# asheptunov/graph-neural-net

Measured on AMD Instinct MI355X. Metric: training samples/sec, 784-300-100-10 MLP batch 128, higher is better.
Workload: dtype f32; 1 GPU; 784-300-100-10 SoftmaxCrossEntropyNeuralNet gradientStep, fp32, batch 128 per GPU (BASELINE configs[1]); global_batch=128, parallelism=dp1, inner_activation=leaky_relu

## Files before the change

graph-neural-net_amd/csrc/abi.hip:

```cpp
#include "handle.h"
#include "confusion_kernel.h"

#include <algorithm>

#include <chrono>
#include "java_random.h"

#include <cmath>
#include <cstdio>
#include <cstdlib>
#include <cstring>

using namespace gnn;
using namespace gnn::host;

namespace {
thread_local std::string g_last_error;
void read_env(gnn_mlp *h) {
    auto is = [](const char *name, const char *val) { const char *e = getenv(name); return e && !strcmp(e, val); };
    h->env_path = is("GNN_MLP_PATH", "generic") ? 1 : is("GNN_MLP_PATH", "nomid4") ? 2 : 0;
    const char *hy = getenv("GNN_MLP_HYBRID");
    h->env_hybrid = hy ? (atoi(hy) & 3) : -1;
    h->env_tail_off = is("GNN_MLP_TAIL", "0");
    h->env_graph = is("GNN_MLP_GRAPH", "1");
    h->env_jit_off = is("GNN_MLP_JIT", "0");
    h->env_static_off = is("GNN_MLP_STATIC", "0");
    h->env_chain_off = is("GNN_MLP_CHAIN", "0");
    h->env_wavek_off = is("GNN_MLP_WAVEK", "0");
    h->env_bf16_dma_off = is("GNN_MLP_BF16_DMA", "0");
    h->env_f32_dma_off = is("GNN_MLP_F32_DMA", "0");
    h->env_bf16_group_off = is("GNN_MLP_BF16_GROUP", "0");
    h->env_rb_off = is("GNN_MLP_ROWBLOCK", "0");
    h->env_defer_off = is("GNN_MLP_DEFER", "0");
    const char *fg = getenv("GNN_MLP_FIRST_GEMM_ROWS");
    if (fg) h->first_gemm_rows = atoi(fg);
    const char *fw = getenv("GNN_MLP_FIRST_WAVEK_ROWS");
    if (fw) h->first_wavek_rows = atoi(fw);
    const char *er = getenv("GNN_MLP_EVAL_ROWS");
    if (er) h->eval_rows_cap = atoi(er);
}
}

namespace gnn {
namespace host {

thread_local ArenaCarve *t_arena = nullptr;

int dev_bytes(void **p, size_t bytes) {
    ArenaCarve *a = t_arena;
    if (a && !a->record) {
        const size_t at = (a->used + 255) & ~(size_t)255;
        if (at + bytes > a->cap) { *p = nullptr; return fail(GNN_ERR_STATE, "group arena exhausted: the members' allocations differ"); }
        *p = a->base + at;
        a->used = at + bytes;
        return GNN_OK;
    }
    HIP_TRY(hipMalloc(p, bytes));
    if (a) a->used = ((a->used + 255) & ~(size_t)255) + bytes;
    return GNN_OK;
}
void dev_release(gnn_mlp *h, void *p) {
    if (!p) return;
    if (h->arena_lo && (size_t)(static_cast<char *>(p) - h->arena_lo) < h->arena_bytes) return;
    (void)hipFree(p);
}
// ... 743 lines not shown
```

graph-neural-net_amd/csrc/group_kernels.h:

```cpp
#pragma once
#include "rowblock_kernel.h"
#include "tile_step_kernel.h"

namespace gnn {

constexpr int GROUP_MAX = 16;

struct GroupArgs {
    const char *arena_lo;
    unsigned long long S;
    const char *idx_lo;
    unsigned long long idx_S;
    int nbx;
    float step_over_b[GROUP_MAX];
    float momentum[GROUP_MAX];
};
struct GroupRows {
    int rows[GROUP_MAX];
    int next_rows[GROUP_MAX];
};

template <class T> __device__ __forceinline__ T *group_rel(T *q, const GroupArgs &g, unsigned long long shift) {
    const unsigned long long d = (unsigned long long)reinterpret_cast<const char *>(q) - (unsigned long long)g.arena_lo;
    return d < g.S ? reinterpret_cast<T *>((unsigned long long)q + shift) : q;
}
__device__ __forceinline__ const int32_t *group_rel_idx(const int32_t *q, const GroupArgs &g, unsigned long long shift) {
    const unsigned long long a = (unsigned long long)reinterpret_cast<const char *>(q);
    const unsigned long long in_idx = 0ull - (unsigned long long)(a - (unsigned long long)g.idx_lo < g.idx_S);
    const unsigned long long in_arena = 0ull - (unsigned long long)(a - (unsigned long long)g.arena_lo < g.S);
    return reinterpret_cast<const int32_t *>(a + ((in_idx & ((unsigned long long)blockIdx.y * g.idx_S)) | (~in_idx & in_arena & shift)));
}
struct GroupIdx { const int32_t *row0, *row, *next; };
template <class T> __device__ __forceinline__ T *group_rel(T *q, const GroupArgs &g, unsigned long long shift, const GroupIdx &) { return group_rel(q, g, shift); }
__device__ __forceinline__ const int32_t *group_rel(const int32_t *q, const GroupArgs &, unsigned long long, const GroupIdx &ix) { return q == ix.row0 ? ix.row : ix.next; }

#define TS_BID blockIdx.x
#define TS_REL(q) group_rel((q), ga, ga_shift, ga_idx)
#define TS_REL_LAYER(L) (L.A = TS_REL(L.A), L.D = TS_REL(L.D), L.W = TS_REL(L.W), L.V = TS_REL(L.V), L.G = TS_REL(L.G))
#define TS_STEP_OVER_B ga.step_over_b[blockIdx.y]
#define TS_MOMENTUM ga.momentum[blockIdx.y]
#define TS_K p.K
#define TS_K_TRUE p.k_true
#define TS_NEXT_ROWS p.next_rows
#define TS_NEXT_K p.next_K
template <int GSRC, int GDST, bool FWD>
__global__ __launch_bounds__(TS_THREADS) void tile_step_group_kernel(TileStepParams p, GroupArgs ga) {
    static_assert(GSRC <= 2, "grouped tile kernels: single-GPU forms only");
    const unsigned long long ga_shift = (unsigned long long)blockIdx.y * ga.S;
    const GroupIdx ga_idx{p.row_idx, group_rel_idx(p.row_idx, ga, ga_shift), group_rel_idx(p.next_idx, ga, ga_shift)};
#include "tile_step_body.inc"
}
template <int GSRC, int GDST, bool FWD>
__global__ __launch_bounds__(TS_THREADS) void tile_step_bf16_group_kernel(TileStepParams p, GroupArgs ga) {
    static_assert(GSRC <= 2, "grouped tile kernels: single-GPU forms only");
    const unsigned long long ga_shift = (unsigned long long)blockIdx.y * ga.S;
    const GroupIdx ga_idx{p.row_idx, group_rel_idx(p.row_idx, ga, ga_shift), group_rel_idx(p.next_idx, ga, ga_shift)};
#include "tile_step_bf16_body.inc"
}
#undef TS_K
#undef TS_K_TRUE
#undef TS_NEXT_ROWS
#undef TS_NEXT_K
#define TS_K ga_K
#define TS_K_TRUE ga_k_true
#define TS_NEXT_ROWS ga_next_rows
#define TS_NEXT_K ga_next_K
#define GNN_GROUP_ROW_COUNTS                                                                      \
    const int ga_k_true = gr.rows[blockIdx.y], ga_K = pad_up(ga_k_true);                          \
    const int ga_next_rows = gr.next_rows[blockIdx.y], ga_next_K = pad_up(ga_next_rows);          \
    (void)ga_k_true; (void)ga_K; (void)ga_next_rows; (void)ga_next_K;
template <int GSRC, int GDST, bool FWD>
__global__ __launch_bounds__(TS_THREADS) void tile_step_group_sized_kernel(TileStepParams p, GroupArgs ga, GroupRows gr) {
    static_assert(GSRC <= 2, "grouped tile kernels: single-GPU forms only");
    const unsigned long long ga_shift = (unsigned long long)blockIdx.y * ga.S;
    const GroupIdx ga_idx{p.row_idx, group_rel_idx(p.row_idx, ga, ga_shift), group_rel_idx(p.next_idx, ga, ga_shift)};
    GNN_GROUP_ROW_COUNTS
#include "tile_step_body.inc"
}
template <int GSRC, int GDST, bool FWD>
__global__ __launch_bounds__(TS_THREADS) void tile_step_bf16_group_sized_kernel(TileStepParams p, GroupArgs ga, GroupRows gr) {
    static_assert(GSRC <= 2, "grouped tile kernels: single-GPU forms only");
    const unsigned long long ga_shift = (unsigned long long)blockIdx.y * ga.S;
    const GroupIdx ga_idx{p.row_idx, group_rel_idx(p.row_idx, ga, ga_shift), group_rel_idx(p.next_idx, ga, ga_shift)};
    GNN_GROUP_ROW_COUNTS
#include "tile_step_bf16_body.inc"
}
#undef TS_BID
#undef TS_REL
#undef TS_REL_LAYER
#undef TS_STEP_OVER_B
#undef TS_MOMENTUM
#undef TS_K
#undef TS_K_TRUE
#undef TS_NEXT_ROWS
#undef TS_NEXT_K
#undef GNN_GROUP_ROW_COUNTS

#define GNN_RB_GROUP_MEMBER(ROWS)                                                                                                  \
    const unsigned long long sh = (unsigned long long)blockIdx.y * g.S;                                                            \
    p.slabs = group_rel(slabs, g, sh); p.row_idx = group_rel_idx(row_idx, g, sh); p.copy_idx = group_rel_idx(copy_idx, g, sh);     \
    _Pragma("unroll")                                                                                                              \
    for (int l = 0; l < MAX_LAYERS; l++) {                                                                                         \
        p.W[l] = group_rel(p.W[l], g, sh); p.act[l] = group_rel(p.act[l], g, sh); p.delta[l] = group_rel(p.delta[l], g, sh);       \
        p.Wb[l] = group_rel(p.Wb[l], g, sh); p.actb[l] = group_rel(p.actb[l], g, sh); p.deltab[l] = group_rel(p.deltab[l], g, sh); \
    }                                                                                                                              \
    p.prob = group_rel(p.prob, g, sh); p.loss = group_rel(p.loss, g, sh); p.label = group_rel(p.label, g, sh);                     \
    p.xcopy = group_rel(p.xcopy, g, sh); p.xcopyb = group_rel(p.xcopyb, g, sh);                                                    \
    p.X = group_rel(p.X, g, sh); p.Xb = group_rel(p.Xb, g, sh);                                                                    \
    if constexpr (BF) {                                                                                                            \
        p.Wb[1] = group_rel(reinterpret_cast<const __bf16 *>(W1), g, sh);                                                          \
        if constexpr (SH::kL > 0) p.Wb[SH::kL - 2] = group_rel(reinterpret_cast<const __bf16 *>(Wlast), g, sh);                    \
    } else {                                                                                                                       \
        p.W[1] = group_rel(W1, g, sh);                                                                                             \
        if constexpr (SH::kL > 0) p.W[SH::kL - 2] = group_rel(Wlast, g, sh);                                                       \
    }                                                                                                                              \
    p.Y = group_rel(Y, g, sh); p.B = (ROWS); p.slab_rows = slab_rows; p.ldy = ldy;                                                 \
    if constexpr (SH::is_static) {                                                                                                 \
        constexpr RbPlan m = SH::make();                                                                                           \
        static_assert(m.ok, "this shape does not fit the row-block kernel");                                                       \
// ... 22 lines not shown
```

graph-neural-net_amd/csrc/handle.h:

```cpp
#pragma once
#include "../../include/gnn_mlp.h"
#include "fused_kernels.h"
#include "gemm_bf16.h"
#include "gemm_wavek.h"
#include "middle4_kernel.h"
#include "rowblock_kernel.h"
#include "tile_step_kernel.h"
#include "group_kernels.h"
#include "group_eval_kernel.h"
#include "kernels.h"
#include "eval_kernels.h"
#include "lookahead.h"
#include "group_sizes.h"
#include "timer_slots.h"

#include <hip/hip_ext.h>
#include <hip/hip_runtime.h>

#include <cstdint>
#include <cstring>
#include <exception>
#include <new>
#include <string>
#include <vector>
// ... 41 lines not shown

    float *DX = nullptr, *DY = nullptr;
    __bf16 *Wb = nullptr;
    std::vector<__bf16 *> actb, deltab;
    __bf16 *DXb = nullptr;
    int64_t dataset_n = 0;

    hipStream_t stream = nullptr, own_stream = nullptr;

    bool fused = false;
    gnn::GradParams grad{};
    int grad_tiles = 0;
    gnn::GradParams grad64{};
    int grad_tiles64 = 0;
    bool mid_generic = false;
    bool mid4 = false;
    gnn::Mid4Params mid4p{};
    size_t mid4_lds_bytes = 0;
    const void *mid4_fn[3] = {nullptr, nullptr, nullptr};
    hipFunction_t mid4_jit[3] = {nullptr, nullptr, nullptr};

    bool rb = false;
    gnn::RbParams rbp{};
    size_t rb_lds_bytes = 0;
    const void *rb_fn = nullptr;
    hipFunction_t rb_jit = nullptr;
    int rb_static = 0;

    bool chain = false;
    gnn::TileStepParams tsp{};
    int ts_tiles = 0, ts_tiles0 = 0;
    uint32_t *ts_map = nullptr, *ts_map0 = nullptr;
    bool ts_map_args = false; uint32_t ts_map_words[2][gnn::TS_MAP_ARGS / 2];
    float *slabs = nullptr;
    int n_slabs = 0;
    std::string plan_note;
    gnn::host::Lookahead la;
    float *xstage[2] = {nullptr, nullptr}; __bf16 *xstage_b[2] = {nullptr, nullptr};
    int specialization = 0;
    bool jit_tried = false;
    int steps_seen = 0;

    hipGraphExec_t tr_exec = nullptr;
    hipGraph_t tr_graph = nullptr;
    int64_t tr_first_batch = -1; int tr_B = 0; int64_t tr_nb = 0; double tr_step = 0, tr_mom = 0;
    const float *tr_dx = nullptr;

    struct PendingUpdate { bool on = false; int B = 0; float step_over_b = 0.f, momentum = 0.f; } pend;
    float *act0_alt = nullptr;
    bool env_defer_off = false;

    static constexpr int kEvalRows = 16384;
    int eval_rows_cap = kEvalRows;
    struct EvalWorkspace {
        int rows = 0;
        std::vector<float *> act;
        float *logits = nullptr, *prob = nullptr, *lossv = nullptr;
        int32_t *labels = nullptr;
    } evalws;

    void *rccl_comm = nullptr; int rccl_ranks = 0, rccl_rank = 0;

    gnn_mlp_group *group = nullptr;
    const gnn::host::GroupLaunch *grp = nullptr;
    char *arena_lo = nullptr; size_t arena_bytes = 0;
    bool shared_dataset = false;
    bool shared_stream = false;

    hipError_t launch_error = hipSuccess;
    const int32_t *cur_idx = nullptr;

    bool timing = false;
    TimerClass timers[5];

    int env_path = 0;
    int env_hybrid = -1;
    bool env_tail_off = false;
    bool env_f32_dma_off = false;
    bool env_bf16_group_off = false;
    bool env_bf16_dma_off = false;
    bool env_wavek_off = false;
    bool env_graph = false;
    bool env_jit_off = false;
    bool env_static_off = false;
    bool env_chain_off = false;
    int first_wavek_rows = 256;
    int first_gemm_rows = 2048;
    bool env_rb_off = false;
};

struct gnn_mlp_group {
    int K = 0, device = 0;
    hipStream_t stream = nullptr;
    char *arena = nullptr;
    size_t S = 0;
    std::vector<gnn_mlp *> m;
    bool grouped = false;
    const void *rb_fn = nullptr;
    const void *rb_fn_sized = nullptr;
    struct EvalPlan { bool ok = false; int mt = 0; gnn::GroupEvalLds lds{}; const void *fn = nullptr, *fn_loss = nullptr; } eval_plan;
    float *eval_ws = nullptr;
    int eval_ws_rows = 0;
    int64_t each_grouped = 0, each_mixed = 0;
    gnn::host::GroupSizes sizes;
};

namespace gnn {
namespace host {

void plan_group_eval(gnn_mlp_group *g);
void free_group_eval(gnn_mlp_group *g);
int enqueue_group_validation(gnn_mlp_group *g, int n, float *loss_rows, int64_t stride);
int enqueue_group_curve_sum(gnn_mlp_group *g, const float *rows, int n_rows, int64_t stride, int n, double *d_out);

int fail(int code, const std::string &msg);
const char *last_error_message();
int check_launches(gnn_mlp *h);
int check_handle(gnn_mlp *h, bool apply_pending = true);
int check_batch(const gnn_mlp *h, int B);
int check_range(const gnn_mlp *h, int64_t first, int B);
// ... 206 lines not shown
```

graph-neural-net_amd/csrc/launch_small.hip:

```cpp
#include "static_shapes.h"
#include "jit.h"

using namespace gnn;
using namespace gnn::host;

namespace gnn {
namespace host {

template <class SH> bool shape_matches(const gnn_mlp *h) {
    constexpr int n = (int)(sizeof(SH::kDims) / sizeof(int));
    if (h->L != n) return false;
    for (int i = 0; i < n; i++) if (h->dims[i] != SH::kDims[i]) return false;
    return true;
}

int static_shape_of(const gnn_mlp *h) {
    if (h->env_static_off) return -1;
    if (shape_matches<ShapeMnistA>(h)) return 0;
    if (shape_matches<ShapeMnistB>(h)) return 1;
    return -1;
}

const void *mid4_function(const gnn_mlp *h, int variant) {
    const bool softmax = h->out_kind == GNN_OUT_SOFTMAX_CE;
// ... 94 lines not shown
void fused_forward(gnn_mlp *h, const float *a0, const float *y, int B, bool backward, bool want_prob,
                   bool want_loss, bool want_label, bool from_slabs, int copy_rows) {
    if (!from_slabs) launch_fwd_first(h, a0, B);
    if (from_slabs && h->rb) {
        RbParams r = h->rbp;
        bind_call(h, r, y, B, want_prob, want_loss, want_label);
        if (copy_rows == RB_COPY_CURRENT && h->cur_idx) {
            r.ldx = h->ld[0]; r.copy_idx = h->cur_idx;
            if (h->dtype == GNN_DTYPE_BF16) { r.Xb = a0_bf16(h, a0); r.xcopyb = h->xstage_b[h->la.xstage_cur]; }
            else { r.X = a0; r.xcopy = h->xstage[h->la.xstage_cur]; }
        } else if (copy_rows == RB_COPY_NEXT && h->la.have_next && h->la.next.idx) {
            r.ldx = h->ld[0]; r.copy_idx = h->la.next.idx;
            if (h->dtype == GNN_DTYPE_BF16) { r.Xb = a0_bf16(h, h->la.next.a0); r.xcopyb = h->xstage_b[h->la.xstage_cur ^ 1]; }
            else { r.X = h->la.next.a0; r.xcopy = h->xstage[h->la.xstage_cur ^ 1]; }
        }
        const bool bf = h->dtype == GNN_DTYPE_BF16;
        const float *hd_W1 = bf ? reinterpret_cast<const float *>(r.Wb[1]) : r.W[1];
        const float *hd_Wl = bf ? reinterpret_cast<const float *>(r.Wb[h->L - 2]) : r.W[h->L - 2];
        void *args[] = {&r.slabs, &hd_W1, &hd_Wl, &r.row_idx, &r.Y, &r.copy_idx, &r.B, &r.slab_rows, &r.ldy, &r};
        const unsigned grid = (unsigned)(pad_up(B) / 4);
        if (h->grp) { launch_rowblock_group(h, B, args); return; }
        launch_instance(h, GNN_K_MIDDLE, h->rb_fn, h->rb_jit, dim3(grid), dim3(RB_NT), h->rb_lds_bytes, args);
        return;
    }
    Mid4Params m4 = h->mid4p;
    for (int l = 1; l < h->L - 1; l++) m4.act[l] = h->act[l];
    bind_call(h, m4, y, B, want_prob, want_loss, want_label);
    m4.n_slabs = h->n_slabs;
    void *args[] = {&m4};
    const int bw = from_slabs ? 2 : backward ? 1 : 0;
    launch_instance(h, GNN_K_MIDDLE, h->mid4_fn[bw], h->mid4_jit[bw], dim3((unsigned)(pad_up(B) / 4)), dim3(1024), h->mid4_lds_bytes, args);
}

struct TileF32 {
    static constexpr bool kPeerForms = true;
    template <int S, int D, bool F> static const void *fn() { return GNN_KERNEL(tile_step_kernel<S, D, F>); }
};
struct TileBf16 {
    static constexpr bool kPeerForms = true;
    template <int S, int D, bool F> static const void *fn() { return GNN_KERNEL(tile_step_bf16_kernel<S, D, F>); }
};

void launch_tile_step(gnn_mlp *h, int gsrc, int gdst, const NextBatch *next, const float *a0, int B, float step_over_b, float momentum,
                      bool staged, const PeerGradients *peers, bool next_staged) {
    TileStepParams t = h->tsp;
    if (peers) {
        for (int r = 0; r < peers->n; r++) t.Gpeer[r] = peers->G[r];
        t.n_peer = peers->n; t.slice = peers->slice; t.Gself = h->G;
    }
    t.layer[0].A = staged ? h->xstage[h->la.xstage_cur] : a0;
    for (int l = 0; l < t.n_layers; l++) t.layer[l].G = h->G + h->w_off[l];
    t.K = pad_up(B); t.k_true = B;
    t.row_idx = staged ? nullptr : h->cur_idx;
    const int stage_dst = h->la.xstage_cur ^ 1;
    if (next && next->idx && !h->rb) { t.stage_out = h->xstage[stage_dst]; t.stage_out_b = h->xstage_b[stage_dst]; }
    t.step_over_b = step_over_b; t.momentum = momentum;
    const bool fwd = next != nullptr;
    if (fwd) { t.An = next->a0; t.ldan = h->ld[0]; t.next_idx = next->idx; t.next_rows = next->B; t.next_K = pad_up(next->B); }
    if (fwd && next_staged) { t.An = h->xstage[stage_dst]; t.next_idx = nullptr; }
    const bool fwd_only = gsrc == 0;
    const dim3 grid(fwd_only ? h->ts_tiles0 : h->ts_tiles), block(TS_THREADS);
    if (fwd_only) t.n_layers = 1;
    t.tile_map = fwd_only ? h->ts_map0 : h->ts_map;
    t.map_in_args = h->ts_map_args ? 1 : 0;
    if (h->ts_map_args) std::memcpy(t.map_words, h->ts_map_words[fwd_only ? 1 : 0], sizeof(t.map_words));
    const int cls = fwd_only ? GNN_K_FWD_GEMM0 : gsrc >= 2 ? GNN_K_UPDATE : GNN_K_GRAD_GEMM0;
    if (h->dtype == GNN_DTYPE_BF16) {
        if (staged) t.Ab[0] = h->xstage_b[h->la.xstage_cur];
        else if (a0) t.Ab[0] = a0_bf16(h, a0);
        if (fwd) t.Anb = next_staged ? h->xstage_b[stage_dst] : a0_bf16(h, next->a0);
    }
    if (h->grp) { launch_tile_step_group(h, gsrc, gdst, fwd, grid.x, t, B); return; }
    const void *fn = h->dtype == GNN_DTYPE_BF16 ? tile_step_instance<TileBf16>(gsrc, gdst, fwd) : tile_step_instance<TileF32>(gsrc, gdst, fwd);
    void *args[] = {&t};
    launch_instance(h, cls, fn, nullptr, grid, block, 0, args);
}

}
}
```

graph-neural-net_amd/csrc/plan.hip:

```cpp
#include "handle.h"

#include <algorithm>

using namespace gnn;
using namespace gnn::host;

namespace gnn {
namespace host {

void plan_fused(gnn_mlp *h) {
    h->fused = false;
    h->mid4 = false;
    h->mid_generic = false;
    h->plan_note.clear();
    if (h->env_path == 1) { h->plan_note = "per-layer GEMMs forced (GNN_MLP_PATH=generic)"; return; }
    const int L = h->L, Lm = L - 1;
    if (L < 3 || L > MAX_LAYERS) { h->plan_note = "fewer than 3 or more than 8 layers: per-layer GEMMs"; return; }
    if (h->dtype != GNN_DTYPE_F32) {
        plan_mid4(h);
        if (h->mid4) { plan_chain(h); plan_rowblock(h); }
        if (!h->chain) h->mid4 = false;
        if (!h->chain && h->plan_note.empty()) h->plan_note = "bf16: the row-block kernel exists for the two-launch path only; per-layer bf16 GEMMs";
        return;
    }
// ... 64 lines not shown
        }
    }
    h->n_slabs = n_slabs;
    TileStepParams &t = h->tsp;
    t.n_layers = L - 1;
    int tiles = 0;
    for (int l = 0; l < L - 1; l++) {
        GradLayer &gl = t.layer[l];
        gl.A = h->act[l]; gl.lda = h->ld[l];
        gl.D = h->delta[l + 1]; gl.ldd = h->ld[l + 1];
        gl.W = h->W + h->w_off[l]; gl.V = h->V + h->w_off[l]; gl.G = h->G + h->w_off[l];
        gl.M = h->ld[l]; gl.N = h->ld[l + 1];
        if (h->dtype == GNN_DTYPE_BF16) { t.Ab[l] = h->actb[l]; t.Db[l] = h->deltab[l + 1]; t.Wb[l] = h->Wb + h->w_off[l]; }
        gl.tiling = make_xcd_tiling((gl.M + TS_TM - 1) / TS_TM, gl.N / TS_TN);
        gl.block_begin = tiles;
        tiles += gl.tiling.blocks();
    }
    {
        TileMapLayer ml[MAX_LAYERS];
        for (int l = 0; l < L - 1; l++) ml[l] = TileMapLayer{h->ld[l], h->ld[l + 1]};
        hipDeviceProp_t prop{};
        int cus = 256;
        if (hipGetDeviceProperties(&prop, h->device) == hipSuccess && prop.multiProcessorCount >= 8) cus = prop.multiProcessorCount;
        else (void)hipGetLastError();
        const std::vector<uint32_t> all = make_tile_map(ml, L - 1, cus / 8, true), first = make_tile_map(ml, 1, cus / 8, true);
        auto upload = [&](const std::vector<uint32_t> &m, uint32_t **dst) {
            if (dev_bytes(reinterpret_cast<void **>(dst), sizeof(uint32_t) * m.size()) != GNN_OK) { *dst = nullptr; return false; }
            return hipMemcpy(*dst, m.data(), sizeof(uint32_t) * m.size(), hipMemcpyHostToDevice) == hipSuccess;
        };
        if (!upload(all, &h->ts_map) || !upload(first, &h->ts_map0)) { give_up("the workgroup -> tile maps could not be placed in device memory"); return; }
        h->ts_tiles = (int)all.size();
        h->ts_tiles0 = (int)first.size();
        h->ts_map_args = pack_tile_map(all, h->ts_map_words[0]) && pack_tile_map(first, h->ts_map_words[1]);
    }
    t.slabs = h->slabs; t.slab_rows = h->cap_rows; t.ldz = h->ld[1];
    h->chain = true;
}

static void slabs_now_hold(gnn_mlp *h, const NextBatch &nb, bool staged_copy, bool by_rowblock = false) {
    h->la.slabs_now_hold(nb, staged_copy && (!h->rb || by_rowblock));
}
void ensure_slabs(gnn_mlp *h, const NextBatch &batch) {
    if (h->la.slabs_hold(batch)) return;
    launch_tile_step(h, 0, 0, &batch, batch.a0, batch.B, 0.f, 0.f);
    slabs_now_hold(h, batch, batch.idx != nullptr);
}
bool update_by_tiles(gnn_mlp *h, int gsrc, float step_over_b, float momentum, const PeerGradients *peers) {
    NextBatch nb{};
    if (!h->chain || !h->la.take_next(&nb)) return false;
    launch_tile_step(h, gsrc, 2, &nb, nullptr, PAD, step_over_b, momentum, false, peers);
    slabs_now_hold(h, nb, nb.idx != nullptr);
    return true;
}

void chain_gradient(gnn_mlp *h, const float *a0, const float *y, int B, bool fused_update, float step_over_b, float momentum, bool resident) {
    Lookahead &la = h->la;
    const NextBatch self{a0, h->cur_idx, B};
    ensure_slabs(h, self);
    const bool have_copy = la.xstage_valid && h->cur_idx != nullptr;
    const bool rb_next = h->rb && fused_update && la.have_next && la.next.idx != nullptr && la.next.B == B && (!h->grp || h->grp->next_same_rows);
    const bool rb_cur = h->rb && !rb_next && !have_copy && h->cur_idx != nullptr;
    const bool staged = have_copy || rb_cur;
    la.step_takes_slabs();
    fused_forward(h, a0, y, B, true, false, false, false, true, rb_next ? RB_COPY_NEXT : rb_cur ? RB_COPY_CURRENT : RB_COPY_NONE);
    NextBatch nb{};
    if (fused_update) {
// ... 212 lines not shown
```

graph-neural-net_amd/csrc/tile_step_bf16_body.inc:

```
    constexpr int LDA = TS_TM + 16;
    constexpr int LDD = TS_TN;
    __shared__ __attribute__((aligned(16))) __bf16 sA[TS_KC * LDA];
    __shared__ __attribute__((aligned(16))) __bf16 sD[TS_KC * LDD];
    __shared__ __attribute__((aligned(16))) __bf16 sW[TS_TM * TS_TN];
    const int t = threadIdx.x, lane = t & 63;
    const int wave = __builtin_amdgcn_readfirstlane(t >> 6);
    const int fr = lane & 15, fg = lane >> 4;

    int li, tm, tn;
    GradLayer L = p.layer[0];
    if (p.map_in_args) {
        const uint32_t w = p.map_words[TS_BID >> 1], e = (TS_BID & 1) ? w >> 16 : w & 0xffffu;
        if (e == 0xffffu) return;
        li = (int)(e & 7u); tm = (int)((e >> 3) & 63u); tn = (int)(e >> 9);
    } else {
        const uint32_t e = p.tile_map[TS_BID];
        if (e == ~0u) return;
        li = (int)(e & 15u); tm = (int)((e >> 4) & 0x3fffu); tn = (int)(e >> 18);
    }
    if (li != 0) L = p.layer[li];
    TS_REL_LAYER(L);
    const int m0 = tm * TS_TM, n0 = tn * TS_TN;
    const bool fwd = FWD && li == 0;
    const __bf16 *Ab = TS_REL(p.Ab[li]), *Db = TS_REL(p.Db[li]);
    const int stage_cols = (L.N / TS_TN) < 8 ? (L.N / TS_TN) : 8;

    const int er = (t >> 6) * 16 + fr, eq = fg;
    const bool e_ok = t < 256 && (m0 + er < L.M);
    const size_t e_off = (size_t)(m0 + er) * L.ldd + n0 + eq * 4;

    bf16x8 va[2], vd;
    const bf16x8 zero8 = {0, 0, 0, 0, 0, 0, 0, 0};
    auto load_grad = [&](int k0, int kc) {
#pragma unroll
        for (int i = 0; i < 2; i++) {
            const int idx = t + i * TS_THREADS, k = idx >> 3, q = idx & 7;
            va[i] = zero8;
            if (k < kc && m0 + q * 8 < L.M) {
                size_t a_row = (size_t)(k0 + k);
                bool live = true;
                if (li == 0 && TS_REL(p.row_idx)) { live = k0 + k < TS_K_TRUE; a_row = live ? (size_t)TS_REL(p.row_idx)[k0 + k] : 0; }
                if (live) va[i] = *reinterpret_cast<const bf16x8 *>(Ab + a_row * L.lda + m0 + q * 8);
            }
        }
        vd = zero8;
        if (t < 256) {
            const int k = t >> 1, q = t & 1;
            if (k < kc) vd = *reinterpret_cast<const bf16x8 *>(Db + (size_t)(k0 + k) * L.ldd + n0 + q * 8);
        }
    };
    const int kc0 = (TS_K < TS_KC) ? TS_K : TS_KC;
    if (GSRC == 1) load_grad(0, kc0);
    float4 w_old = make_float4(0.f, 0.f, 0.f, 0.f), v_old = w_old, g_in = w_old;
    if (e_ok) {
        if (GDST == 2 || FWD) w_old = *reinterpret_cast<const float4 *>(L.W + e_off);
        if (GDST == 2) v_old = *reinterpret_cast<const float4 *>(L.V + e_off);
    }
    if (GSRC >= 2) g_in = ts_gradient_in<GSRC>(p, L, e_off, e_ok);
    s16x4 vn[2][2];
    int next_row0 = wave * 16 + fr;
    if (fwd && TS_REL(p.next_idx) && next_row0 < TS_NEXT_ROWS) next_row0 = TS_REL(p.next_idx)[next_row0];
    auto load_next = [&](int b0) {
        const int b = b0 + wave * 16 + fr;
        const bool live = b < TS_NEXT_ROWS;
        const size_t row = live ? (b0 == 0 ? (size_t)next_row0 : TS_REL(p.next_idx) ? (size_t)TS_REL(p.next_idx)[b] : (size_t)b) : 0;
        const __bf16 *src = TS_REL(p.Anb) + row * p.ldan + m0 + 4 * fg;
#pragma unroll
        for (int kb = 0; kb < 2; kb++)
#pragma unroll
            for (int hh = 0; hh < 2; hh++) {
                vn[kb][hh] = (s16x4){0, 0, 0, 0};
                if (live && m0 + kb * 32 + hh * 16 + 4 * fg < L.M) vn[kb][hh] = *reinterpret_cast<const s16x4 *>(src + kb * 32 + hh * 16);
            }
    };
// ... 71 lines not shown
```

graph-neural-net_amd/csrc/tile_step_body.inc:

```
    constexpr int NW = TS_THREADS / 64, NT = TS_THREADS, RPW = 1;
    constexpr int LDA = TS_TM + 16;
    constexpr int LDD = TS_TN;
    constexpr int LDW = TS_TN + 4;
    __shared__ __attribute__((aligned(16))) float sA[TS_KC * LDA];
    __shared__ __attribute__((aligned(16))) float sD[TS_KC * LDD];
    __shared__ __attribute__((aligned(16))) float sW[TS_TM * LDW];
    const int t = threadIdx.x, lane = t & 63;
    const int wave = __builtin_amdgcn_readfirstlane(t >> 6);
    const int fr = lane & 15, fq = lane >> 4;

    int li, tm, tn;
    GradLayer L = p.layer[0];
    if (p.map_in_args) {
        const uint32_t w = p.map_words[TS_BID >> 1], e = (TS_BID & 1) ? w >> 16 : w & 0xffffu;
        if (e == 0xffffu) return;
        li = (int)(e & 7u); tm = (int)((e >> 3) & 63u); tn = (int)(e >> 9);
    } else {
        const uint32_t e = p.tile_map[TS_BID];
        if (e == ~0u) return;
        li = (int)(e & 15u); tm = (int)((e >> 4) & 0x3fffu); tn = (int)(e >> 18);
    }
    if (li != 0) L = p.layer[li];
    TS_REL_LAYER(L);
    const int m0 = tm * TS_TM, n0 = tn * TS_TN;
    const bool fwd = FWD && li == 0;

    const int er = (t >> 6) * 16 + fr, eq = fq;
    const bool e_ok = t < 256 && (m0 + er < L.M);
    const size_t e_off = (size_t)(m0 + er) * L.ldd + n0 + eq * 4;

    float4 va[4 * RPW], vd[RPW];
    const int kc0 = (TS_K < TS_KC) ? TS_K : TS_KC;
    const bool interior = (m0 + TS_TM <= L.M) && (TS_K >= TS_KC) && !(li == 0 && TS_REL(p.row_idx)) &&
                          (unsigned long long)TS_KC * (unsigned)(L.lda > L.ldd ? L.lda : L.ldd) < 0xffffffffull;
    if (GSRC == 1 && interior) {
#pragma unroll
        for (int i = 0; i < 4 * RPW; i++) {
            const int idx = t + i * NT, k = idx >> 4, q = idx & 15;
            va[i] = *reinterpret_cast<const float4 *>(L.A + ((unsigned)k * (unsigned)L.lda + m0 + q * 4));
        }
#pragma unroll
        for (int i = 0; i < RPW; i++) {
            const int idx = t + i * NT;
            vd[i] = *reinterpret_cast<const float4 *>(L.D + ((unsigned)(idx >> 2) * (unsigned)L.ldd + n0 + (idx & 3) * 4));
        }
    } else if (GSRC == 1) {
#pragma unroll
        for (int i = 0; i < 4 * RPW; i++) {
            const int idx = t + i * NT, k = idx >> 4, q = idx & 15;
            va[i] = make_float4(0.f, 0.f, 0.f, 0.f);
            if (k < kc0 && m0 + q * 4 < L.M) {
                size_t a_row = (size_t)k;
                bool live = true;
                if (li == 0 && TS_REL(p.row_idx)) { live = k < TS_K_TRUE; a_row = live ? (size_t)TS_REL(p.row_idx)[k] : 0; }
                if (live) va[i] = *reinterpret_cast<const float4 *>(L.A + a_row * L.lda + m0 + q * 4);
            }
        }
#pragma unroll
        for (int i = 0; i < RPW; i++) {
            const int idx = t + i * NT, k = idx >> 2, q = idx & 3;
            vd[i] = make_float4(0.f, 0.f, 0.f, 0.f);
            if (k < kc0) vd[i] = *reinterpret_cast<const float4 *>(L.D + (size_t)k * L.ldd + n0 + q * 4);
        }
    }
    float4 w_old = make_float4(0.f, 0.f, 0.f, 0.f), v_old = w_old, g_in = w_old;
    if (e_ok) {
        if (GDST == 2 || FWD) w_old = *reinterpret_cast<const float4 *>(L.W + e_off);
        if (GDST == 2) v_old = *reinterpret_cast<const float4 *>(L.V + e_off);
    }
    if (GSRC >= 2) g_in = ts_gradient_in<GSRC>(p, L, e_off, e_ok);
    const bool next_plain = interior && fwd && !TS_REL(p.next_idx) && TS_NEXT_ROWS >= TS_KC && (unsigned long long)TS_KC * (unsigned)p.ldan < 0xffffffffull;
    const bool next_gather = (m0 + TS_TM <= L.M) && fwd && TS_REL(p.next_idx) && TS_NEXT_ROWS >= TS_KC;
    const int stage_cols = (L.N / TS_TN) < 8 ? (L.N / TS_TN) : 8;
    f32x4 vn[RPW][4];
    int next_row0[RPW];
#pragma unroll
    for (int g = 0; g < RPW; g++) {
        next_row0[g] = (wave + g * NW) * 16 + fr;
        if (fwd && TS_REL(p.next_idx) && next_row0[g] < TS_NEXT_ROWS) next_row0[g] = TS_REL(p.next_idx)[next_row0[g]];
    }
    auto load_next = [&](int b0) {
#pragma unroll
        for (int g = 0; g < RPW; g++) {
            const int b = b0 + (wave + g * NW) * 16 + fr;
            if (b0 == 0 && next_plain) {
                const float *src = TS_REL(p.An) + ((unsigned)b * (unsigned)p.ldan + m0 + 4 * fq);
#pragma unroll
                for (int c = 0; c < 4; c++) vn[g][c] = *reinterpret_cast<const f32x4 *>(src + c * 16);
                continue;
            }
            if (b0 == 0 && next_gather) {
                const float *src = TS_REL(p.An) + ((size_t)next_row0[g] * p.ldan + m0 + 4 * fq);
#pragma unroll
                for (int c = 0; c < 4; c++) vn[g][c] = *reinterpret_cast<const f32x4 *>(src + c * 16);
                continue;
            }
            const bool live = b < TS_NEXT_ROWS;
            const size_t row = live ? (b0 == 0 ? (size_t)next_row0[g] : TS_REL(p.next_idx) ? (size_t)TS_REL(p.next_idx)[b] : (size_t)b) : 0;
            const float *src = TS_REL(p.An) + row * p.ldan + m0 + 4 * fq;
#pragma unroll
            for (int c = 0; c < 4; c++) {
                vn[g][c] = (f32x4){0.f, 0.f, 0.f, 0.f};
                if (live && m0 + c * 16 + 4 * fq < L.M) vn[g][c] = *reinterpret_cast<const f32x4 *>(src + c * 16);
            }
        }
    };
// ... 6 lines not shown
            const int kc = (TS_K - k0 < TS_KC) ? TS_K - k0 : TS_KC;
            if (k0) {
                __syncthreads();
#pragma unroll
                for (int i = 0; i < 4 * RPW; i++) {
                    const int idx = t + i * NT, k = idx >> 4, q = idx & 15;
                    va[i] = make_float4(0.f, 0.f, 0.f, 0.f);
                    if (k < kc && m0 + q * 4 < L.M) {
                        size_t a_row = (size_t)(k0 + k);
                        bool live = true;
                        if (li == 0 && TS_REL(p.row_idx)) { live = k0 + k < TS_K_TRUE; a_row = live ? (size_t)TS_REL(p.row_idx)[k0 + k] : 0; }
                        if (live) va[i] = *reinterpret_cast<const float4 *>(L.A + a_row * L.lda + m0 + q * 4);
                    }
                }
#pragma unroll
                for (int i = 0; i < RPW; i++) {
                    const int idx = t + i * NT, k = idx >> 2, q = idx & 3;
                    vd[i] = make_float4(0.f, 0.f, 0.f, 0.f);
                    if (k < kc) vd[i] = *reinterpret_cast<const float4 *>(L.D + (size_t)(k0 + k) * L.ldd + n0 + q * 4);
                }
            }
#pragma unroll
            for (int i = 0; i < 4 * RPW; i++) {
                const int idx = t + i * NT, k = idx >> 4, q = idx & 15;
                *reinterpret_cast<float4 *>(&sA[k * LDA + q * 4]) = va[i];
            }
#pragma unroll
            for (int i = 0; i < RPW; i++) {
                const int idx = t + i * NT;
                *reinterpret_cast<float4 *>(&sD[(idx >> 2) * LDD + (idx & 3) * 4]) = vd[i];
            }
            __syncthreads();
            if (k0 == 0) {
                if (fwd) load_next(0);
            }
            if (wave < 4) {
                const float *ap = &sA[fq * LDA + wave * 16 + fr];
                const float *dp = &sD[fq * LDD + fr];
                int kk = 0;
                if (kc == TS_KC) {
                    float a[2][8], d[2][8];
#pragma unroll
                    for (int j = 0; j < 8; j++) { a[0][j] = ap[(4 * j) * LDA]; d[0][j] = dp[(4 * j) * LDD]; }
#pragma unroll
                    for (int trip = 0; trip < TS_KC / 32; trip++) {
                        const int cur = trip & 1;
                        if (trip + 1 < TS_KC / 32) {
#pragma unroll
                            for (int j = 0; j < 8; j++) { a[cur ^ 1][j] = ap[(32 * (trip + 1) + 4 * j) * LDA]; d[cur ^ 1][j] = dp[(32 * (trip + 1) + 4 * j) * LDD]; }
                        }
                        __builtin_amdgcn_sched_barrier(0);
#pragma unroll
                        for (int j = 0; j < 8; j += 2) {
                            acc0 = __builtin_amdgcn_mfma_f32_16x16x4f32(d[cur][j], a[cur][j], acc0, 0, 0, 0);
                            acc1 = __builtin_amdgcn_mfma_f32_16x16x4f32(d[cur][j + 1], a[cur][j + 1], acc1, 0, 0, 0);
                        }
                        __builtin_amdgcn_sched_barrier(0);
                    }
                    kk = TS_KC;
                }
                for (; kk + 32 <= kc; kk += 32) {
                    float a[8], d[8];
#pragma unroll
                    for (int j = 0; j < 8; j++) { a[j] = ap[(kk + 4 * j) * LDA]; d[j] = dp[(kk + 4 * j) * LDD]; }
#pragma unroll
                    for (int j = 0; j < 8; j += 2) {
                        acc0 = __builtin_amdgcn_mfma_f32_16x16x4f32(d[j], a[j], acc0, 0, 0, 0);
                        acc1 = __builtin_amdgcn_mfma_f32_16x16x4f32(d[j + 1], a[j + 1], acc1, 0, 0, 0);
                    }
                }
                for (; kk < kc; kk += 4)
                    acc0 = __builtin_amdgcn_mfma_f32_16x16x4f32(dp[kk * LDD], ap[kk * LDA], acc0, 0, 0, 0);
            }
        }
        const f32x4 acc = acc0 + acc1;
        g = make_float4(acc[0], acc[1], acc[2], acc[3]);
    }

    float4 w_new = w_old;
    if (GDST == 1) {
        if (e_ok) *reinterpret_cast<float4 *>(L.G + e_off) = g;
    } else if (GDST == 2) {
        float4 adj;
        adj.x = sgd_adj(TS_STEP_OVER_B, g.x, TS_MOMENTUM, v_old.x);
        adj.y = sgd_adj(TS_STEP_OVER_B, g.y, TS_MOMENTUM, v_old.y);
        adj.z = sgd_adj(TS_STEP_OVER_B, g.z, TS_MOMENTUM, v_old.z);
        adj.w = sgd_adj(TS_STEP_OVER_B, g.w, TS_MOMENTUM, v_old.w);
        w_new = make_float4(w_old.x - adj.x, w_old.y - adj.y, w_old.z - adj.z, w_old.w - adj.w);
        if (e_ok) {
            ts_store16(L.W + e_off, (f32x4){w_new.x, w_new.y, w_new.z, w_new.w});
            ts_store16(L.V + e_off, (f32x4){adj.x, adj.y, adj.z, adj.w});
        }
    }
    if (!fwd) return;

    if (t < 256) *reinterpret_cast<float4 *>(&sW[er * LDW + eq * 4]) = e_ok ? w_new : make_float4(0.f, 0.f, 0.f, 0.f);
    __syncthreads();
    float *slab = TS_REL(p.slabs) + (size_t)tm * p.slab_rows * p.ldz;
    const float *wcol = &sW[(4 * fq) * LDW + fr];
    float wv[4][4];
#pragma unroll
    for (int c = 0; c < 4; c++)
#pragma unroll
        for (int j = 0; j < 4; j++) wv[c][j] = wcol[(c * 16 + j) * LDW];
    for (int b0 = 0; b0 < TS_NEXT_K; b0 += TS_KC) {
        if (b0) load_next(b0);
#pragma unroll
        for (int g = 0; g < RPW; g++) {
            const int wr = (wave + g * NW) * 16;
            if (TS_REL(p.stage_out) && b0 + wr < TS_NEXT_K && (((b0 + wr) >> 4) % stage_cols) == tn % stage_cols && tn < stage_cols) {
                float *dst = TS_REL(p.stage_out) + (size_t)(b0 + wr + fr) * p.ldan + m0 + 4 * fq;
#pragma unroll
                for (int c = 0; c < 4; c++)
                    if (m0 + c * 16 + 4 * fq < L.M) *reinterpret_cast<f32x4 *>(dst + c * 16) = vn[g][c];
            }
            if (b0 + wr < TS_NEXT_K) {
                f32x4 z0 = {0.f, 0.f, 0.f, 0.f}, z1 = {0.f, 0.f, 0.f, 0.f};
#pragma unroll
                for (int c = 0; c < 4; c++) {
#pragma unroll
                    for (int j = 0; j < 4; j++) {
                        if (c & 1) z1 = __builtin_amdgcn_mfma_f32_16x16x4f32(wv[c][j], vn[g][c][j], z1, 0, 0, 0);
                        else z0 = __builtin_amdgcn_mfma_f32_16x16x4f32(wv[c][j], vn[g][c][j], z0, 0, 0, 0);
                    }
                }
                const f32x4 z = z0 + z1;
                ts_store16(slab + (size_t)(b0 + wr + fr) * p.ldz + n0 + 4 * fq, z);
            }
        }
    }
```

graph-neural-net_amd/csrc/tile_step_kernel.h:

```cpp
#pragma once
#include "fused_kernels.h"
#include "gemm_bf16.h"
#ifndef __HIPCC_RTC__
#include <algorithm>
#include <vector>
#endif

namespace gnn {

constexpr int TS_TM = 64, TS_TN = 16, TS_THREADS = 512, TS_KC = 128;
constexpr int TS_MAX_SLABS = 16;
constexpr int TS_MAX_PEERS = 16;
constexpr int TS_MAP_ARGS = 640;

struct TileStepParams {
    GradLayer layer[MAX_LAYERS];
    int n_layers;
    int K, k_true;
    float step_over_b, momentum;
    const int32_t *row_idx;
    const float *An; int ldan;
    const int32_t *next_idx;
    int next_rows, next_K;
    float *slabs;
// ... 39 lines not shown
    }
    size_t slots = 0;
    for (int x = 0; x < 8; x++) slots = per_xcd[x].size() > slots ? per_xcd[x].size() : slots;
    std::vector<uint32_t> map(slots * 8, ~0u);
    for (int x = 0; x < 8; x++) {
        std::vector<T> &v = per_xcd[x];
        const int n = (int)v.size(), k = n > cus_per_xcd ? (n - cus_per_xcd < n / 2 ? n - cus_per_xcd : n / 2) : 0;
        std::vector<int> order(n);
        for (int i = 0; i < n; i++) order[i] = i;
        std::stable_sort(order.begin(), order.end(), [&](int a, int b) { return v[a].w < v[b].w; });
        std::vector<char> is_light(n, 0);
        std::vector<uint32_t> seq;
        for (int i = k; i < 2 * k; i++) { seq.push_back(v[order[i]].e); is_light[order[i]] = 1; }
        for (int i = 0; i < k; i++) is_light[order[i]] = 1;
        for (int i = 0; i < n; i++) if (!is_light[i]) seq.push_back(v[i].e);
        for (int i = 0; i < k; i++) seq.push_back(v[order[i]].e);
        for (int j = 0; j < n; j++) map[(size_t)j * 8 + x] = seq[j];
    }
    return map;
}
inline bool pack_tile_map(const std::vector<uint32_t> &map, uint32_t (&words)[TS_MAP_ARGS / 2]) {
    if (map.size() > (size_t)TS_MAP_ARGS) return false;
    for (uint32_t &w : words) w = 0xffffffffu;
    for (size_t i = 0; i < map.size(); i++) {
        uint32_t e16 = 0xffffu;
        if (map[i] != ~0u) {
            const uint32_t li = map[i] & 15u, tm = (map[i] >> 4) & 0x3fffu, tn = map[i] >> 18;
            if (li > 7 || tm > 63 || tn > 126) return false;
            e16 = li | tm << 3 | tn << 9;
        }
        words[i >> 1] = (i & 1) ? ((words[i >> 1] & 0x0000ffffu) | e16 << 16) : ((words[i >> 1] & 0xffff0000u) | e16);
    }
    return true;
}

__device__ __forceinline__ void ts_mfma_result(f32x4 &v) { asm volatile("s_nop 7\n\ts_nop 7\n\ts_nop 3" : "+v"(v)); }
__device__ __forceinline__ void ts_store16(float *dst, f32x4 v) {
    asm volatile("global_store_dwordx4 %0, %1, off sc1\n\ts_nop 1" ::"v"(dst), "v"(v) : "memory");
}

template <int GSRC> __device__ __forceinline__ float4 ts_gradient_in(const TileStepParams &p, const GradLayer &L, size_t e_off, bool e_ok) {
    float4 g = make_float4(0.f, 0.f, 0.f, 0.f);
    if (!e_ok) return g;
    if (GSRC == 2) {
        g = *reinterpret_cast<const float4 *>(L.G + e_off);
    } else if (GSRC == 3) {
        const size_t off = (size_t)(L.G - p.Gself) + e_off;
        g = *reinterpret_cast<const float4 *>(p.Gpeer[0] + off);
#pragma unroll
        for (int r = 1; r < TS_MAX_PEERS; r++) {
            if (r < p.n_peer) {
                const float4 o = *reinterpret_cast<const float4 *>(p.Gpeer[r] + off);
                g.x += o.x; g.y += o.y; g.z += o.z; g.w += o.w;
            }
        }
    } else if (GSRC == 4) {
        const size_t off = (size_t)(L.G - p.Gself) + e_off;
        const unsigned owner = (unsigned)off / p.slice;
        const float *src = p.Gpeer[0];
#pragma unroll
        for (int r = 1; r < TS_MAX_PEERS; r++) src = (owner == (unsigned)r) ? p.Gpeer[r] : src;
        g = *reinterpret_cast<const float4 *>(src + off);
    }
    return g;
}


#define TS_BID blockIdx.x
#define TS_REL(q) (q)
#define TS_REL_LAYER(L)
#define TS_STEP_OVER_B p.step_over_b
#define TS_MOMENTUM p.momentum
#define TS_K p.K
#define TS_K_TRUE p.k_true
#define TS_NEXT_ROWS p.next_rows
#define TS_NEXT_K p.next_K
template <int GSRC, int GDST, bool FWD>
__global__ __launch_bounds__(TS_THREADS) void tile_step_kernel(TileStepParams p) {
#include "tile_step_body.inc"
}


template <int GSRC, int GDST, bool FWD>
__global__ __launch_bounds__(TS_THREADS) void tile_step_bf16_kernel(TileStepParams p) {
#include "tile_step_bf16_body.inc"
}
#undef TS_BID
#undef TS_REL
#undef TS_REL_LAYER
#undef TS_STEP_OVER_B
#undef TS_MOMENTUM
#undef TS_K
#undef TS_K_TRUE
#undef TS_NEXT_ROWS
#undef TS_NEXT_K

}
```

Before: 9.873 million samples/s.

## Pass head-tile geometry as scalar kernel args and defer W/V loads

Adds a 'tile head' fast path. Each block of the first-layer tile-step kernel computes its tile coordinates arithmetically from packed geometry words passed as scalar kernel arguments, instead of reading the tile map and the layer struct from the parameter block. First-layer A/D/W/V pointers, leading dimensions, M and K are also passed as separate scalar arguments. In the f32 kernel the old-weight and velocity loads are moved after the first LDS stage sync, to shorten the prologue's critical path. This adds host-side geometry validation, more kernel template instances and an env switch, and it risks wrong tile coordinates from the float reciprocal division.

```diff
diff --git a/graph-neural-net_amd/csrc/abi.hip b/graph-neural-net_amd/csrc/abi.hip
--- a/graph-neural-net_amd/csrc/abi.hip
+++ b/graph-neural-net_amd/csrc/abi.hip
@@ -31,6 +31,7 @@
     h->env_f32_dma_off = is("GNN_MLP_F32_DMA", "0");
     h->env_bf16_group_off = is("GNN_MLP_BF16_GROUP", "0");
     h->env_rb_off = is("GNN_MLP_ROWBLOCK", "0");
+    h->env_tile_head_off = is("GNN_MLP_TILE_HEAD", "0");
     h->env_defer_off = is("GNN_MLP_DEFER", "0");
     const char *fg = getenv("GNN_MLP_FIRST_GEMM_ROWS");
     if (fg) h->first_gemm_rows = atoi(fg);
diff --git a/graph-neural-net_amd/csrc/group_kernels.h b/graph-neural-net_amd/csrc/group_kernels.h
--- a/graph-neural-net_amd/csrc/group_kernels.h
+++ b/graph-neural-net_amd/csrc/group_kernels.h
@@ -34,6 +34,10 @@
 template <class T> __device__ __forceinline__ T *group_rel(T *q, const GroupArgs &g, unsigned long long shift, const GroupIdx &) { return group_rel(q, g, shift); }
 __device__ __forceinline__ const int32_t *group_rel(const int32_t *q, const GroupArgs &, unsigned long long, const GroupIdx &ix) { return q == ix.row0 ? ix.row : ix.next; }
 
+#define TS_HEAD_PROLOGUE 0
+#define TS_DEFER_WV 0
+#define TS_HAS_ROW_IDX TS_REL(p.row_idx)
+#define TS_STAGE_N L.N
 #define TS_BID blockIdx.x
 #define TS_REL(q) group_rel((q), ga, ga_shift, ga_idx)
 #define TS_REL_LAYER(L) (L.A = TS_REL(L.A), L.D = TS_REL(L.D), L.W = TS_REL(L.W), L.V = TS_REL(L.V), L.G = TS_REL(L.G))
@@ -85,6 +89,10 @@
     GNN_GROUP_ROW_COUNTS
 #include "tile_step_bf16_body.inc"
 }
+#undef TS_HEAD_PROLOGUE
+#undef TS_DEFER_WV
+#undef TS_HAS_ROW_IDX
+#undef TS_STAGE_N
 #undef TS_BID
 #undef TS_REL
 #undef TS_REL_LAYER
diff --git a/graph-neural-net_amd/csrc/handle.h b/graph-neural-net_amd/csrc/handle.h
--- a/graph-neural-net_amd/csrc/handle.h
+++ b/graph-neural-net_amd/csrc/handle.h
@@ -97,6 +97,7 @@
     int ts_tiles = 0, ts_tiles0 = 0;
     uint32_t *ts_map = nullptr, *ts_map0 = nullptr;
     bool ts_map_args = false; uint32_t ts_map_words[2][gnn::TS_MAP_ARGS / 2];
+    gnn::TileHead ts_head[2] = {{0, 0}, {0, 0}};
     float *slabs = nullptr;
     int n_slabs = 0;
     std::string plan_note;
@@ -151,6 +152,7 @@
     bool env_chain_off = false;
     int first_wavek_rows = 256;
     int first_gemm_rows = 2048;
+    bool env_tile_head_off = false;
     bool env_rb_off = false;
 };
 
diff --git a/graph-neural-net_amd/csrc/launch_small.hip b/graph-neural-net_amd/csrc/launch_small.hip
--- a/graph-neural-net_amd/csrc/launch_small.hip
+++ b/graph-neural-net_amd/csrc/launch_small.hip
@@ -150,13 +150,13 @@
     launch_instance(h, GNN_K_MIDDLE, h->mid4_fn[bw], h->mid4_jit[bw], dim3((unsigned)(pad_up(B) / 4)), dim3(1024), h->mid4_lds_bytes, args);
 }
 
-struct TileF32 {
+template <bool HEAD> struct TileF32 {
     static constexpr bool kPeerForms = true;
-    template <int S, int D, bool F> static const void *fn() { return GNN_KERNEL(tile_step_kernel<S, D, F>); }
+    template <int S, int D, bool F> static const void *fn() { return GNN_KERNEL(tile_step_kernel<S, D, F, HEAD, HEAD>); }
 };
-struct TileBf16 {
+template <bool HEAD> struct TileBf16 {
     static constexpr bool kPeerForms = true;
-    template <int S, int D, bool F> static const void *fn() { return GNN_KERNEL(tile_step_bf16_kernel<S, D, F>); }
+    template <int S, int D, bool F> static const void *fn() { return GNN_KERNEL(tile_step_bf16_kernel<S, D, F, HEAD>); }
 };
 
 void launch_tile_step(gnn_mlp *h, int gsrc, int gdst, const NextBatch *next, const float *a0, int B, float step_over_b, float momentum,
@@ -189,8 +189,14 @@
         if (fwd) t.Anb = next_staged ? h->xstage_b[stage_dst] : a0_bf16(h, next->a0);
     }
     if (h->grp) { launch_tile_step_group(h, gsrc, gdst, fwd, grid.x, t, B); return; }
-    const void *fn = h->dtype == GNN_DTYPE_BF16 ? tile_step_instance<TileBf16>(gsrc, gdst, fwd) : tile_step_instance<TileF32>(gsrc, gdst, fwd);
-    void *args[] = {&t};
+    const bool bf = h->dtype == GNN_DTYPE_BF16, head = !h->env_tile_head_off;
+    const void *fn = bf ? (head ? tile_step_instance<TileBf16<true>>(gsrc, gdst, fwd) : tile_step_instance<TileBf16<false>>(gsrc, gdst, fwd))
+                        : (head ? tile_step_instance<TileF32<true>>(gsrc, gdst, fwd) : tile_step_instance<TileF32<false>>(gsrc, gdst, fwd));
+    const GradLayer &l0 = t.layer[0];
+    const float *hd_A = bf ? reinterpret_cast<const float *>(t.Ab[0]) : l0.A, *hd_D = bf ? reinterpret_cast<const float *>(t.Db[0]) : l0.D;
+    int hd_Kr = t.K | (t.row_idx ? 1 : 0);
+    TileHead hd = h->ts_head[fwd_only ? 1 : 0];
+    void *args[] = {&hd_A, &hd_D, &t.layer[0].W, &t.layer[0].V, &t.layer[0].lda, &t.layer[0].ldd, &t.layer[0].M, &hd_Kr, &hd.geo, &hd.kx, &t};
     launch_instance(h, cls, fn, nullptr, grid, block, 0, args);
 }
 
diff --git a/graph-neural-net_amd/csrc/plan.hip b/graph-neural-net_amd/csrc/plan.hip
--- a/graph-neural-net_amd/csrc/plan.hip
+++ b/graph-neural-net_amd/csrc/plan.hip
@@ -120,6 +120,8 @@
         h->ts_tiles = (int)all.size();
         h->ts_tiles0 = (int)first.size();
         h->ts_map_args = pack_tile_map(all, h->ts_map_words[0]) && pack_tile_map(first, h->ts_map_words[1]);
+        h->ts_head[0] = make_tile_head(ml, all);
+        h->ts_head[1] = make_tile_head(ml, first);
     }
     t.slabs = h->slabs; t.slab_rows = h->cap_rows; t.ldz = h->ld[1];
     h->chain = true;
diff --git a/graph-neural-net_amd/csrc/tile_step_bf16_body.inc b/graph-neural-net_amd/csrc/tile_step_bf16_body.inc
--- a/graph-neural-net_amd/csrc/tile_step_bf16_body.inc
+++ b/graph-neural-net_amd/csrc/tile_step_bf16_body.inc
@@ -9,6 +9,13 @@
 
     int li, tm, tn;
     GradLayer L = p.layer[0];
+#if TS_HEAD_PROLOGUE
+    const bool regular = TS_HEAD && ts_head_tile(hd_geo, hd_kx, (int)TS_BID, tm, tn);
+    if (regular) {
+        li = 0;
+        L.W = hd_W; L.V = hd_V; L.lda = hd_lda; L.ldd = hd_ldd; L.M = hd_M;
+    } else
+#endif
     if (p.map_in_args) {
         const uint32_t w = p.map_words[TS_BID >> 1], e = (TS_BID & 1) ? w >> 16 : w & 0xffffu;
         if (e == 0xffffu) return;
@@ -22,8 +29,12 @@
     TS_REL_LAYER(L);
     const int m0 = tm * TS_TM, n0 = tn * TS_TN;
     const bool fwd = FWD && li == 0;
+#if TS_HEAD_PROLOGUE
+    const __bf16 *Ab = regular ? reinterpret_cast<const __bf16 *>(hd_A) : p.Ab[li], *Db = regular ? reinterpret_cast<const __bf16 *>(hd_D) : p.Db[li];
+#else
     const __bf16 *Ab = TS_REL(p.Ab[li]), *Db = TS_REL(p.Db[li]);
-    const int stage_cols = (L.N / TS_TN) < 8 ? (L.N / TS_TN) : 8;
+#endif
+    const int stage_cols = (TS_STAGE_N / TS_TN) < 8 ? (TS_STAGE_N / TS_TN) : 8;
 
     const int er = (t >> 6) * 16 + fr, eq = fg;
     const bool e_ok = t < 256 && (m0 + er < L.M);
@@ -39,7 +50,7 @@
             if (k < kc && m0 + q * 8 < L.M) {
                 size_t a_row = (size_t)(k0 + k);
                 bool live = true;
-                if (li == 0 && TS_REL(p.row_idx)) { live = k0 + k < TS_K_TRUE; a_row = live ? (size_t)TS_REL(p.row_idx)[k0 + k] : 0; }
+                if (li == 0 && TS_HAS_ROW_IDX) { live = k0 + k < TS_K_TRUE; a_row = live ? (size_t)TS_REL(p.row_idx)[k0 + k] : 0; }
                 if (live) va[i] = *reinterpret_cast<const bf16x8 *>(Ab + a_row * L.lda + m0 + q * 8);
             }
         }
diff --git a/graph-neural-net_amd/csrc/tile_step_body.inc b/graph-neural-net_amd/csrc/tile_step_body.inc
--- a/graph-neural-net_amd/csrc/tile_step_body.inc
+++ b/graph-neural-net_amd/csrc/tile_step_body.inc
@@ -8,9 +8,17 @@
     const int t = threadIdx.x, lane = t & 63;
     const int wave = __builtin_amdgcn_readfirstlane(t >> 6);
     const int fr = lane & 15, fq = lane >> 4;
+    TS_STAMP(0);
 
     int li, tm, tn;
     GradLayer L = p.layer[0];
+#if TS_HEAD_PROLOGUE
+    const bool regular = TS_HEAD && ts_head_tile(hd_geo, hd_kx, (int)TS_BID, tm, tn);
+    if (regular) {
+        li = 0;
+        L.A = hd_A; L.D = hd_D; L.W = hd_W; L.V = hd_V; L.lda = hd_lda; L.ldd = hd_ldd; L.M = hd_M;
+    } else
+#endif
     if (p.map_in_args) {
         const uint32_t w = p.map_words[TS_BID >> 1], e = (TS_BID & 1) ? w >> 16 : w & 0xffffu;
         if (e == 0xffffu) return;
@@ -31,7 +39,7 @@
 
     float4 va[4 * RPW], vd[RPW];
     const int kc0 = (TS_K < TS_KC) ? TS_K : TS_KC;
-    const bool interior = (m0 + TS_TM <= L.M) && (TS_K >= TS_KC) && !(li == 0 && TS_REL(p.row_idx)) &&
+    const bool interior = (m0 + TS_TM <= L.M) && (TS_K >= TS_KC) && !(li == 0 && TS_HAS_ROW_IDX) &&
                           (unsigned long long)TS_KC * (unsigned)(L.lda > L.ldd ? L.lda : L.ldd) < 0xffffffffull;
     if (GSRC == 1 && interior) {
 #pragma unroll
@@ -63,15 +71,17 @@
             if (k < kc0) vd[i] = *reinterpret_cast<const float4 *>(L.D + (size_t)k * L.ldd + n0 + q * 4);
         }
     }
+    TS_STAMP(1);
+    constexpr bool defer_wv = TS_DEFER_WV && GSRC == 1;
     float4 w_old = make_float4(0.f, 0.f, 0.f, 0.f), v_old = w_old, g_in = w_old;
-    if (e_ok) {
+    if (!defer_wv && e_ok) {
         if (GDST == 2 || FWD) w_old = *reinterpret_cast<const float4 *>(L.W + e_off);
         if (GDST == 2) v_old = *reinterpret_cast<const float4 *>(L.V + e_off);
     }
     if (GSRC >= 2) g_in = ts_gradient_in<GSRC>(p, L, e_off, e_ok);
     const bool next_plain = interior && fwd && !TS_REL(p.next_idx) && TS_NEXT_ROWS >= TS_KC && (unsigned long long)TS_KC * (unsigned)p.ldan < 0xffffffffull;
     const bool next_gather = (m0 + TS_TM <= L.M) && fwd && TS_REL(p.next_idx) && TS_NEXT_ROWS >= TS_KC;
-    const int stage_cols = (L.N / TS_TN) < 8 ? (L.N / TS_TN) : 8;
+    const int stage_cols = (TS_STAGE_N / TS_TN) < 8 ? (TS_STAGE_N / TS_TN) : 8;
     f32x4 vn[RPW][4];
     int next_row0[RPW];
 #pragma unroll
@@ -144,6 +154,11 @@
             }
             __syncthreads();
             if (k0 == 0) {
+                TS_STAMP(2);
+                if (defer_wv && e_ok) {
+                    if (GDST == 2 || FWD) w_old = *reinterpret_cast<const float4 *>(L.W + e_off);
+                    if (GDST == 2) v_old = *reinterpret_cast<const float4 *>(L.V + e_off);
+                }
                 if (fwd) load_next(0);
             }
             if (wave < 4) {
@@ -204,6 +219,7 @@
             ts_store16(L.V + e_off, (f32x4){adj.x, adj.y, adj.z, adj.w});
         }
     }
+    TS_STAMP(3);
     if (!fwd) return;
 
     if (t < 256) *reinterpret_cast<float4 *>(&sW[er * LDW + eq * 4]) = e_ok ? w_new : make_float4(0.f, 0.f, 0.f, 0.f);
@@ -241,3 +257,4 @@
             }
         }
     }
+    TS_STAMP(3);
diff --git a/graph-neural-net_amd/csrc/tile_step_kernel.h b/graph-neural-net_amd/csrc/tile_step_kernel.h
--- a/graph-neural-net_amd/csrc/tile_step_kernel.h
+++ b/graph-neural-net_amd/csrc/tile_step_kernel.h
@@ -95,6 +95,46 @@
         words[i >> 1] = (i & 1) ? ((words[i >> 1] & 0x0000ffffu) | e16 << 16) : ((words[i >> 1] & 0xffff0000u) | e16);
     }
     return true;
+}
+
+struct TileHead { uint32_t geo, kx; };
+__host__ __device__ __forceinline__ bool ts_head_tile(uint32_t geo, uint32_t kx, int id, int &tm, int &tn) {
+    const int rm = (int)(geo & 63u), rn = (int)((geo >> 6) & 255u), xs = (int)((geo >> 14) & 3u);
+    const int full_m = (int)((geo >> 16) & 127u), tiles_n = (int)(geo >> 23);
+    const int x = id & 7, j = (id >> 3) - (int)((kx >> (4 * x)) & 15u);
+    const int r0 = (x >> xs) * rm, c0 = (x & ((1 << xs) - 1)) * rn;
+    const int h = full_m - r0 < rm ? full_m - r0 : rm, w = tiles_n - c0 < rn ? tiles_n - c0 : rn;
+    if (j < 0 || h <= 0 || w <= 0 || j >= h * w) return false;
+#if defined(__HIP_DEVICE_COMPILE__)
+    const int q = (int)(((float)j + 0.5f) * __builtin_amdgcn_rcpf((float)w));
+#else
+    const int q = (int)(((float)j + 0.5f) * (1.0f / (float)w));
+#endif
+    tm = r0 + q; tn = c0 + (j - q * w);
+    return true;
+}
+inline TileHead make_tile_head(const TileMapLayer *layers, const std::vector<uint32_t> &map, bool force_mismatch = false) {
+    const int tiles_m = (layers[0].M + TS_TM - 1) / TS_TM, tiles_n = layers[0].N / TS_TN;
+    int full_m = 0;
+    for (int tm = 0; tm < tiles_m; tm++) if (layers[0].M - tm * TS_TM > TS_TM / 2) full_m = tm + 1;
+    if (full_m == 0 || map.empty() || map.size() % 8 != 0) return TileHead{0, 0};
+    const XcdTiling rect = make_xcd_tiling(full_m, tiles_n);
+    if (rect.rm > 63 || rect.rn > 255 || rect.xs > 3 || full_m > 127 || tiles_n > 511) return TileHead{0, 0};
+    TileHead hd{(uint32_t)rect.rm | (uint32_t)rect.rn << 6 | (uint32_t)rect.xs << 14 | (uint32_t)full_m << 16 | (uint32_t)tiles_n << 23, 0};
+    for (int x = 0; x < 8; x++) {
+        const int r0 = (x >> rect.xs) * rect.rm, c0 = (x & (rect.xn - 1)) * rect.rn;
+        if (r0 >= full_m || c0 >= tiles_n) continue;
+        size_t k = 0;
+        while (k * 8 < map.size() && map[k * 8 + x] != ((uint32_t)r0 << 4 | (uint32_t)c0 << 18)) k++;
+        if (k > 15) return TileHead{0, 0};
+        hd.kx |= (uint32_t)k << (4 * x);
+    }
+    if (force_mismatch) hd.kx ^= 1u;
+    for (size_t id = 0; id < map.size(); id++) {
+        int tm = 0, tn = 0;
+        if (ts_head_tile(hd.geo, hd.kx, (int)id, tm, tn) && map[id] != ((uint32_t)tm << 4 | (uint32_t)tn << 18)) return TileHead{0, 0};
+    }
+    return hd;
 }
 
 __device__ __forceinline__ void ts_mfma_result(f32x4 &v) { asm volatile("s_nop 7\n\ts_nop 7\n\ts_nop 3" : "+v"(v)); }
@@ -129,25 +169,39 @@
 }
 
 
+#define GNN_TS_HEAD_PARAMS const float *hd_A, const float *hd_D, float *hd_W, float *hd_V, int hd_lda, int hd_ldd, int hd_M, int hd_Kr, uint32_t hd_geo, uint32_t hd_kx
+#define TS_HEAD_PROLOGUE 1
+#define TS_HEAD HEAD
+#define TS_DEFER_WV DEFER_WV
+#ifndef TS_STAMP
+#define TS_STAMP(slot)
+#endif
 #define TS_BID blockIdx.x
 #define TS_REL(q) (q)
 #define TS_REL_LAYER(L)
 #define TS_STEP_OVER_B p.step_over_b
 #define TS_MOMENTUM p.momentum
-#define TS_K p.K
+#define TS_K (HEAD ? (hd_Kr & ~1) : p.K)
 #define TS_K_TRUE p.k_true
+#define TS_HAS_ROW_IDX (HEAD ? (hd_Kr & 1) != 0 : p.row_idx != nullptr)
+#define TS_STAGE_N p.layer[0].N
 #define TS_NEXT_ROWS p.next_rows
 #define TS_NEXT_K p.next_K
-template <int GSRC, int GDST, bool FWD>
-__global__ __launch_bounds__(TS_THREADS) void tile_step_kernel(TileStepParams p) {
+template <int GSRC, int GDST, bool FWD, bool HEAD = true, bool DEFER_WV = true>
+__global__ __launch_bounds__(TS_THREADS) void tile_step_kernel(GNN_TS_HEAD_PARAMS, TileStepParams p) {
 #include "tile_step_body.inc"
 }
 
 
-template <int GSRC, int GDST, bool FWD>
-__global__ __launch_bounds__(TS_THREADS) void tile_step_bf16_kernel(TileStepParams p) {
+template <int GSRC, int GDST, bool FWD, bool HEAD = true>
+__global__ __launch_bounds__(TS_THREADS) void tile_step_bf16_kernel(GNN_TS_HEAD_PARAMS, TileStepParams p) {
 #include "tile_step_bf16_body.inc"
 }
+#undef TS_HEAD_PROLOGUE
+#undef TS_HEAD
+#undef TS_DEFER_WV
+#undef TS_HAS_ROW_IDX
+#undef TS_STAGE_N
 #undef TS_BID
 #undef TS_REL
 #undef TS_REL_LAYER
```

Result: faster. 10.03 million samples/s, median of 6 (+1.6%).
